# yamiel-abreu/distributed-pytorch-training

Hardware: AMD Instinct MI355X
Metric: images/sec (whole node) ResNet-50 bf16 training (higher is better)
Workload: dtype bf16

## Files before the change

csrc/bindings.cpp:

```cpp
#include <ATen/ATen.h>
#include <c10/hip/HIPGuard.h>
#include <c10/hip/HIPStream.h>
#include <torch/extension.h>

#include "kernels/kernels.h"
#include "host_comm.h"
#include "pg_comm.h"
#include "rccl_comm.h"
#include "watchdog.h"
#include "reducer.h"

namespace py = pybind11;
using at::Tensor;

namespace {

hipStream_t cur_stream(const Tensor& t) {
  return c10::hip::getCurrentHIPStream(t.device().index()).stream();
}

dpt::WireType wire_of(const Tensor& t) {
  switch (t.scalar_type()) {
    case at::kFloat: return dpt::WireType::kF32;
    case at::kBFloat16: return dpt::WireType::kBF16;
// ... 1216 lines not shown
  m.def("bias_grad16", &bias_grad16, py::arg("grad"), py::arg("out_kind"));
  m.def("sum_partials", &sum_partials, py::arg("part"), py::arg("out_kind"));
  m.def("colsum_rows", &colsum_rows, py::arg("part"), py::arg("out_kind"));
  m.def("maxpool_fwd", &maxpool_fwd, py::arg("x"), py::arg("k"), py::arg("stride"), py::arg("pad"),
        py::arg("bn_coef") = py::none());
  m.def("gap_bwd", &gap_bwd, py::arg("g"), py::arg("H"), py::arg("W"), py::arg("dtype"));
  m.def("gap_bwd_bnr", &gap_bwd_bnr, py::arg("g"), py::arg("y"), py::arg("x"), py::arg("mean"));
  m.def("maxpool_bwd", &maxpool_bwd, py::arg("grad_output"), py::arg("idx"), py::arg("H"), py::arg("W"),
        py::arg("k"), py::arg("stride"), py::arg("pad"), py::arg("grad_output2") = py::none(),
        py::arg("bn_x") = py::none(), py::arg("bn_mean") = py::none(), py::arg("bn_coef") = py::none());
  m.def("conv_fwd", &conv_fwd, py::arg("x"), py::arg("w"), py::arg("stride"), py::arg("pad"), py::arg("want_stats"),
        py::arg("out_h") = 0, py::arg("out_w") = 0);
  m.def("space_to_depth2", &space_to_depth2, py::arg("x"), py::arg("out_f16") = false);
  m.def("conv_wgrad", &conv_wgrad, py::arg("grad_output"), py::arg("x"), py::arg("weight_shape"), py::arg("stride"),
        py::arg("pad"), py::arg("fp32_out"), py::arg("target_blocks") = 0);
  m.def("conv_f32_fwd", &conv_f32_fwd, py::arg("x"), py::arg("w"), py::arg("stride"), py::arg("pad"),
        py::arg("split") = false);
  m.def("conv_f32_dgrad", &conv_f32_dgrad, py::arg("grad_output"), py::arg("w"), py::arg("stride"), py::arg("pad"),
        py::arg("H"), py::arg("W"), py::arg("split") = false);
  m.def("conv_f32_wgrad", &conv_f32_wgrad, py::arg("grad_output"), py::arg("x"), py::arg("weight_shape"),
        py::arg("stride"), py::arg("pad"), py::arg("split") = false);
  m.def("im2col", &im2col, py::arg("x"), py::arg("R"), py::arg("S"), py::arg("stride"), py::arg("pad"), py::arg("Kp"));
  m.def("attn_fwd", &attn_fwd, py::arg("qkv"), py::arg("heads"), py::arg("scale"));
  m.def("attn_set_bwd_split", &dpt::attn_set_bwd_split, py::arg("on"));
  m.def("attn_bwd", &attn_bwd, py::arg("qkv"), py::arg("out"), py::arg("grad_output"), py::arg("lse"),
        py::arg("heads"), py::arg("scale"));
  m.def("attn_stream_fwd", &attn_stream_fwd, py::arg("qkv"), py::arg("heads"), py::arg("scale"));
  m.def("attn_stream_bwd", &attn_stream_bwd, py::arg("qkv"), py::arg("out"), py::arg("grad_output"), py::arg("lse"),
        py::arg("heads"), py::arg("scale"));
  m.def("attn_stream_tiles", &attn_stream_tiles,
        "(queries per workgroup, keys per chunk, query rows per backward chunk) of the streaming attention kernels");
  m.def("conv_set_variant", &dpt::conv_set_variant, py::arg("variant"));
  m.def("bn_set_skip_finalize", &dpt::bn_set_skip_finalize, py::arg("on"),
        "measurement only: skip every BatchNorm finalize launch (wrong values; timing upper bound)");
  m.def("conv_set_splitk_policy", &dpt::conv_set_splitk_policy, py::arg("tiles"), py::arg("eager_tiles"),
        py::arg("eager_min_k"), py::arg("target"), "split-K thresholds (A/B knob; <= 0 keeps a value)");
  m.def("conv_set_big", &dpt::conv_set_big, py::arg("on"));
  m.def("conv_set_halo", &dpt::conv_set_halo, py::arg("on"));
  m.def("conv_set_breg", &dpt::conv_set_breg, py::arg("mode"));
  m.def("conv_set_wgrad_stages", &dpt::conv_set_wgrad_stages, py::arg("mode"));
  m.def("conv_get_breg", &dpt::conv_get_breg);
  m.def("conv_set_streamk", &dpt::conv_set_streamk, py::arg("mode"), py::arg("eff") = 0.0);
  m.def("conv_get_streamk", &dpt::conv_get_streamk);
  m.def("conv_sk_prepare", &dpt::conv_sk_prepare);
  m.def("conv_sk_errors", &dpt::conv_sk_errors);
  m.def("conv_sk_blocks", &dpt::conv_sk_blocks, py::arg("tiles"), py::arg("nk"), py::arg("bn"), py::arg("mode"));
  m.def("conv_set_wgrad_target", &dpt::conv_set_wgrad_target, py::arg("blocks"));
  m.def("conv_set_wgrad_halo", &dpt::conv_set_wgrad_halo, py::arg("mode"));
  m.def("conv_fwd_splits", [](int64_t M, int Cout, int64_t K, bool graph) {
          return dpt::conv_fwd_splits_for(M, Cout, K, graph);
        }, py::arg("M"), py::arg("Cout"), py::arg("K"), py::arg("graph") = false);
  m.def("conv_set_splitk", &dpt::conv_set_splitk, py::arg("mode"));
  m.def("conv_get_splitk", &dpt::conv_get_splitk);
  m.def("conv_set_fwd_shape_policy", &dpt::conv_set_fwd_shape_policy, py::arg("bits"));
  m.def("conv_dgrad", &conv_dgrad, py::arg("grad_output"), py::arg("w"), py::arg("pad"));
  m.def("conv_dgrad_bnstats", &conv_dgrad_bnstats, py::arg("grad_output"), py::arg("w"), py::arg("pad"),
        py::arg("bn_x"), py::arg("bn_mean"), py::arg("bn_coef"), py::arg("bn_y") = py::none(),
        py::arg("bn_res") = py::none(), py::arg("w_flipped") = py::none(), py::arg("bn_x2") = py::none(),
        py::arg("bn_mean2") = py::none(), py::arg("wgrad_reduce") = nullptr, py::arg("bn_mask") = py::none(),
        py::arg("bn_res_s2") = false);
  m.def("conv_wt_flip_multi", &conv_wt_flip_multi, py::arg("ws"));
  m.def("conv_dgrad_preflipped", &conv_dgrad_preflipped, py::arg("grad_output"), py::arg("w_flipped"), py::arg("pad"),
        py::arg("wgrad_reduce") = nullptr);
  m.def("bn_bwd_partials", &bn_bwd_partials, py::arg("grad_output"), py::arg("x"), py::arg("weight"), py::arg("mean"),
        py::arg("invstd"), py::arg("coef"), py::arg("p1"), py::arg("p2"), py::arg("want_dparams"),
        py::arg("from_dz") = false);
  m.def("conv_dgrad_s2", &conv_dgrad_s2, py::arg("grad_output"), py::arg("w"), py::arg("pad"), py::arg("H"),
        py::arg("W"), py::arg("bn_x") = py::none(), py::arg("bn_mean") = py::none(), py::arg("bn_coef") = py::none(),
        py::arg("wgrad_reduce") = nullptr, py::arg("compact") = false);
  m.def("conv_dgrad_flip", &conv_dgrad_flip, py::arg("grad_output"), py::arg("w"), py::arg("pad"),
        py::arg("wgrad_reduce") = nullptr);
  py::class_<PendingReduce, PendingReducePtr>(m, "PendingWgradReduce")
      .def_property_readonly("done", &PendingReduce::done)
      .def_property_readonly("splits", [](const PendingReduce& p) { return p.r.splits; });
  m.def("conv_wgrad_deferred", &conv_wgrad_deferred, py::arg("grad_output"), py::arg("x"), py::arg("weight_shape"),
        py::arg("stride"), py::arg("pad"));
  m.def("conv_reduce_flush", &conv_reduce_flush, py::arg("pending"));
  m.def("rccl_version", []() { return std::string(dpt::rccl_version_string()); });

  py::class_<dpt::Collective, std::shared_ptr<dpt::Collective>>(m, "Collective")
      .def("all_reduce", [](dpt::Collective& c, Tensor t, bool on_current_stream) {
             TORCH_CHECK(t.is_cuda() && t.is_contiguous(), "all_reduce needs a contiguous GPU tensor");
             c10::hip::HIPGuard guard(t.device().index());
             hipStream_t s = cur_stream(t);
             c.all_reduce(t.data_ptr(), (size_t)t.numel(), wire_of(t), on_current_stream ? s : c.stream());
           }, py::arg("tensor"), py::arg("on_current_stream") = true)
      .def("broadcast", [](dpt::Collective& c, Tensor t, int root) {
             TORCH_CHECK(t.is_cuda() && t.is_contiguous(), "broadcast needs a contiguous GPU tensor");
             c10::hip::HIPGuard guard(t.device().index());
             c.broadcast(t.data_ptr(), (size_t)t.numel(), wire_of(t), root, cur_stream(t));
           }, py::arg("tensor"), py::arg("root") = 0)
      .def("abort", &dpt::Collective::abort)
      .def("destroy", &dpt::Collective::destroy)
      .def("check", &dpt::Collective::check)
      .def_property_readonly("kind", &dpt::Collective::kind)
      .def_property_readonly("ops", &dpt::Collective::ops)
      .def_property_readonly("sequence_hash", &dpt::Collective::sequence_hash)
      .def_property_readonly("rank", &dpt::Collective::rank)
      .def_property_readonly("world_size", &dpt::Collective::world_size)
      .def_property_readonly("device", &dpt::Collective::device)
      .def("track", [](dpt::Collective& c) {
             c10::hip::HIPGuard guard(c.device());
             c.track(c10::hip::getCurrentHIPStream(c.device()).stream());
           }, "hand the watchdog a completion marker for the work enqueued on the current stream")
      .def("_test_spin", [](dpt::Collective& c, double ms, bool on_current_stream) {
             TORCH_CHECK(ms >= 0 && ms <= 20000, "spin: 0..20000 ms");
// ... 87 lines not shown
```

csrc/kernels/conv_kernels.hip:

```cpp
#include <algorithm>
#include <cmath>
#include <cstdlib>
#include <mutex>
#include <stdexcept>
#include <type_traits>

#include "carry.h"
#include "gelu.h"
#include "common.h"
#include "kernels.h"
#include "mfma.h"

namespace dpt {


#ifndef DPT_WGRAD_WAVES
#define DPT_WGRAD_WAVES 4
#endif
#ifndef DPT_CONV_HALF_EPI
#define DPT_CONV_HALF_EPI 0
#endif

namespace conv {

// ... 29 lines not shown
}
template <bool F16>
__device__ __forceinline__ uint32_t cpack(f32x2_t v) {
  if constexpr (F16) return __builtin_bit_cast(uint32_t, __builtin_convertvector(v, f16x2_t));
  else return __builtin_bit_cast(uint32_t, __builtin_convertvector(v, bf16x2_t));
}
template <bool F16>
__device__ __forceinline__ float cunpack(uint32_t u, int h) {
  if constexpr (F16) return (float)__builtin_bit_cast(_Float16, (uint16_t)(h ? (u >> 16) : (u & 0xffffu)));
  else return __uint_as_float(h ? (u & 0xffff0000u) : (u << 16));
}

struct ConvSk {
  float* part = nullptr;
  unsigned* flags = nullptr;
  unsigned* err = nullptr;
  int G = 0;
  uint32_t part_bytes = 0;
};

struct ConvFwdArgs {
  const uint16_t* x = nullptr;
  const uint16_t* w = nullptr;
  uint16_t* y = nullptr;
  float* psum = nullptr;
  float* psq = nullptr;
  int N = 0, H = 0, W = 0, C = 0, Ho = 0, Wo = 0, Cout = 0, R = 0, S = 0, stride = 0, pad = 0;
  int64_t M = 0;
  int m_tiles = 0, n_tiles = 0;
  int mt256 = 0;
  const uint16_t* bnx = nullptr;
  const float* bn_mean = nullptr;
  const float* bn_coef = nullptr;
  float* bp1 = nullptr;
  float* bp2 = nullptr;
  const uint16_t* bny = nullptr;
  const uint16_t* bnres = nullptr;
  const uint8_t* bnmask = nullptr;
  int rHo = 0, rWo = 0;
  const uint16_t* bias16 = nullptr;
  const uint16_t* bnx2 = nullptr;
  const float* bn_mean2 = nullptr;
  float* bp3 = nullptr;
  int Rw = 0, Sw = 0, tr0 = 0, trs = 0, ts0 = 0, tss = 0;
  int oH = 0, oW = 0, oph = 0, opw = 0;
  int bp_ld = 0, bp_off = 0;
  int f16 = 0;
  float* part = nullptr;
  int splits = 1, kps = 0;
  ReduceCarry red;
  ConvSk sk;
};


template <int N>
__device__ __forceinline__ void vmcnt_wait() {
  asm volatile("s_waitcnt vmcnt(%0)" ::"n"(N) : "memory");
}

template <int RB>
__device__ __forceinline__ bf16x8_t wg_frag(const unsigned char* img, int krow0, int col0, int lane) {
  return tr_frag<RB, false>(img, krow0, col0, lane);
}

__device__ __attribute__((aligned(64))) uint4 g_conv_zero16[4];

template <int BMT, int BN, int STAGES, bool LDSEPI, bool BKN, bool STATS = true, bool BNB = false,
          bool BNR = false, bool REMAP = false, bool ZSIB = false, bool BNR2 = false, bool F16 = false,
          int NT = conv::kThreads, bool SPLIT = false, bool HALO = false, int HB = 1, bool SK = false,
          bool DGELU = false, bool BREG = false, bool RS2 = false>
__global__ __launch_bounds__(NT, (SK || BREG) ? 4 : 2) void conv_fwd_kernel(ConvFwdArgs p) {
  static_assert(!RS2 || (BNR && !BNR2 && !REMAP && LDSEPI && !HALO && !BREG), "RS2 config");
  using namespace conv;
  constexpr int BM = BMT;
  constexpr int NW = NT / 64;
  constexpr int WCOL = BREG ? 32 : 64;
  constexpr int WN = BN / WCOL;
  constexpr int WM = NW / WN;
  constexpr int MI = BM / (WM * 32);
  constexpr int NI = WCOL / 32;
  static_assert(WM * WN == NW && MI >= 1 && MI * WM * 32 == BM, "conv_fwd_kernel: bad wave tiling");
  constexpr int A_PER_T = BM * 8 / NT;
  constexpr int B_PER_T = BN * 8 / NT;
  static_assert(!HALO || (BMT == 128 && STAGES == 1 && !BKN && !SPLIT && NT == conv::kThreads), "HALO config");
  static_assert(!SK || (STAGES == 1 && !HALO && !SPLIT && LDSEPI && !BNR2 && NT == conv::kThreads), "SK config");
  static_assert(!DGELU || (BNB && !BNR && !STATS && !REMAP && LDSEPI && !SK), "DGELU config");
  static_assert(!BREG || (BMT == 128 && STAGES == 1 && LDSEPI && !BKN && !SPLIT && !SK && HB == 1 &&
                          NT == conv::kThreads && (BN == 128 || BN == 64)), "BREG config");
  constexpr int HROWS = 136;
  static_assert(HB == 1 || (HALO && HB == 3), "HB");
  constexpr int A_BYTES = (HALO ? HROWS : BM) * kRowBytes, B_BYTES = BN * kRowBytes;
  constexpr int STAGE = A_BYTES + (BREG ? 0 : HB * B_BYTES);
  constexpr int NSTAGE = BREG ? 2 : STAGES;
  constexpr int C_STRIDE = BN * 2 + 16;
  constexpr int RED = 2 * WM * BN * 4;
  constexpr int ZROW = NSTAGE * STAGE;
  constexpr int LDS_MAIN = NSTAGE * STAGE + (HALO ? kRowBytes : 0);
  constexpr bool HALF = DPT_CONV_HALF_EPI && LDSEPI && BM == 128 && NT == conv::kThreads && MI * 32 <= 64 && !BNB &&
                        !SPLIT;
  constexpr int EROWS = HALF ? 64 : BM;
  constexpr int LDS_EPI = (LDSEPI ? EROWS * C_STRIDE : 0) + RED;
  constexpr int LDS = LDS_MAIN > LDS_EPI ? LDS_MAIN : LDS_EPI;
  __shared__ __attribute__((aligned(16))) unsigned char lds[LDS];
  if constexpr (NT == conv::kThreads) {
    if (p.red.blocks) {
      const int nconv = (int)gridDim.x - p.red.blocks;
      if ((int)blockIdx.x >= nconv) {
        carry_reduce(p.red, (int)blockIdx.x - nconv, lds);
        return;
      }
    }
  }

  const int tid = threadIdx.x, lane = tid & 63, wid = tid >> 6;
  const int wm = wid / WN, wn = wid % WN;
  const int tiles = (BM == 256 ? p.mt256 : p.m_tiles) * p.n_tiles;
  const int nk_all = (int)((int64_t)p.R * p.S * p.C / BK);

  auto tile_body = [&](const int mt, const int nt, const int sp, const int ks0, const int ks1, const int sk_role,
                       const int sk_slot, const int sk_c0, const int sk_c1) {
  const int tid = SK ? conv::opaque_v((int)threadIdx.x) : (int)threadIdx.x, lane = tid & 63;
  const int wid = SK ? __builtin_amdgcn_readfirstlane(tid >> 6) : tid >> 6;
  const int wm = wid / WN, wn = wid % WN;
  const int64_t m0 = (int64_t)mt * BM;
  const int n0 = nt * BN;

  int hi0[A_PER_T], wi0[A_PER_T], aoff[A_PER_T];
  const int64_t HoWo = (int64_t)p.Ho * p.Wo;
#pragma unroll
  for (int i = 0; i < A_PER_T; ++i) {
    const int arow = (wid * A_PER_T + i) * 8 + (lane >> 3);
    const int achunk = (lane & 7) ^ ((arow >> 1) & 7);
    const int64_t m = m0 + arow;
    if (m < p.M) {
      const int64_t n = m / HoWo;
      const int rem = (int)(m - n * HoWo);
      const int ho = rem / p.Wo, wo = rem - ho * p.Wo;
      hi0[i] = ho * p.stride - p.pad;
      wi0[i] = wo * p.stride - p.pad + (p.C < BK ? achunk * 8 / p.C : 0);
      aoff[i] = (int)(((n * p.H + hi0[i]) * (int64_t)p.W + wo * p.stride - p.pad) * p.C + achunk * 8);
    } else {
      hi0[i] = -(1 << 28);
      wi0[i] = 0;
      aoff[i] = 0;
    }
  }
  const int64_t Kg = (int64_t)p.R * p.S * p.C;
  int woff[B_PER_T];
  constexpr int RBK = BN * 2;
  constexpr int KN_RPI = 1024 / RBK;
#pragma unroll
  for (int i = 0; i < B_PER_T; ++i) {
    if (BKN) {
      const int krow = (wid * B_PER_T + i) * KN_RPI + lane / (RBK / 16);
      const int kchunk = wg_slot<RBK>(krow, lane % (RBK / 16));
      woff[i] = krow * p.Rw * p.Sw * p.Cout + n0 + kchunk * 8;
    } else {
      const int brow = (wid * B_PER_T + i) * 8 + (lane >> 3);
      const int bchunk = (lane & 7) ^ ((brow >> 1) & 7);
      woff[i] = (int)((n0 + brow) * Kg) + bchunk * 8;
    }
  }
  constexpr uint32_t kOOB = 0xFFFFFF00u;
  const __amdgpu_buffer_rsrc_t rx = __builtin_amdgcn_make_buffer_rsrc(
// ... 652 lines not shown
      if (tid < BN) {
        float a = 0.f, b = 0.f, c3 = 0.f;
#pragma unroll
        for (int w = 0; w < NW; ++w) {
          a += bred[(w * NS3) * BN + tid];
          b += bred[(w * NS3 + 1) * BN + tid];
          if (two) c3 += bred[(w * NS3 + 2) * BN + tid];
        }
        constexpr int SUBB = BM / 128;
        const int64_t pc = DGELU ? (int64_t)mt * p.Cout + n0 + tid
                                 : (int64_t)(n0 + tid) * p.bp_ld + p.bp_off + (int64_t)mt * SUBB;
        p.bp1[pc] = a;
        if (!DGELU) p.bp2[pc] = b;
        if (two) p.bp3[pc] = c3;
        if (SUBB == 2 && ((int64_t)mt * 2 + 1) * 128 < p.M) {
          p.bp1[pc + 1] = 0.f;
          if (!DGELU) p.bp2[pc + 1] = 0.f;
          if (two) p.bp3[pc + 1] = 0.f;
        }
      }
    }
  }
  };

  if constexpr (SK) {
    const uint32_t g = (uint32_t)p.sk.G >> 3, nk = (uint32_t)nk_all;
    const uint32_t x = blockIdx.x & 7, i = blockIdx.x >> 3;
    const uint32_t t_lo = (uint32_t)tiles * x / 8, t_hi = (uint32_t)tiles * (x + 1) / 8;
    const uint32_t I = (t_hi - t_lo) * nk;
    const uint32_t s0 = I * i / g, s1 = I * (i + 1) / g;
    const uint32_t f1 = min(s1, (s0 / nk + 1) * nk);
    const uint32_t nseg = s1 > s0 ? 1u + (s1 > f1 ? (s1 - 1) / nk - f1 / nk + 1 : 0u) : 0u;
    for (uint32_t q = 0; q < nseg; ++q) {
      const uint32_t b0 = q + 1 == nseg ? s0 : f1 + q * nk;
      const uint32_t tl = b0 / nk;
      const uint32_t b1 = min(s1, (tl + 1) * nk);
      const int k0 = (int)(b0 - tl * nk), k1 = (int)(b1 - tl * nk);
      int role = 0, c0 = 0, c1 = -1;
      if (k0 > 0 && k1 == nk_all) {
        role = 2;
        const uint32_t it0 = tl * nk;
        uint32_t c = it0 * g / I;
        while (c + 1 < i && I * (c + 1) / g <= it0) ++c;
        while (c > 0 && I * c / g > it0) --c;
        c0 = (int)(x + 8 * c);
        c1 = (int)blockIdx.x - 8;
      } else if (k1 < nk_all) {
        role = 1;
      }
      if (q > 0) __syncthreads();
      const int t = (int)(t_lo + tl);
      tile_body(t / p.n_tiles, t % p.n_tiles, 0, k0, k1, role, (int)blockIdx.x, c0, c1);
    }
  } else {
    const int nsplit = SPLIT ? p.splits : 1;
    const int bid0 = conv::xcd_remap(blockIdx.x, tiles * nsplit);
    const int sp = SPLIT ? bid0 % nsplit : 0;
    const int bid = SPLIT ? bid0 / nsplit : bid0;
    const int ks0 = SPLIT ? sp * p.kps : 0;
    const int ks1 = SPLIT ? min(nk_all, ks0 + p.kps) : nk_all;
    tile_body(bid / p.n_tiles, bid % p.n_tiles, sp, ks0, ks1, 0, 0, 0, -1);
  }
}

constexpr int kSplitRows = 16;
template <bool STATS, bool BNB, bool BNR, bool BNR2, bool REMAP, bool ZSIB, bool F16, bool RS2 = false>
__global__ __launch_bounds__(256) void conv_split_epilogue_kernel(ConvFwdArgs p) {
  static_assert(!RS2 || (BNR && !BNR2 && !REMAP), "RS2 config");
  const int rb = blockIdx.x, cgb = blockIdx.y, cols = gridDim.x;
  const int tid = threadIdx.x, lane = tid & 63, wid = tid >> 6;
  const int oc = tid & 7, orow = (tid >> 3) & 15, half = tid >> 7;
  const int c0 = cgb * 64 + oc * 8;
  const int64_t MC = p.M * p.Cout;
  const int64_t m = (int64_t)rb * kSplitRows + orow;
  const bool live = m < p.M;
  const int64_t poff = (live ? m : 0) * p.Cout + c0;
  int64_t grow = live ? m : 0;
  int oy = 0, ox = 0;
  if (REMAP) {
    const int64_t hw = (int64_t)p.Ho * p.Wo, img = grow / hw, rem = grow - img * hw;
    const int a = (int)(rem / p.Wo), b = (int)(rem - (int64_t)a * p.Wo);
    oy = 2 * a + p.oph;
    ox = 2 * b + p.opw;
    grow = (img * p.oH + oy) * p.oW + ox;
  }
  const int64_t off = grow * p.Cout + c0;
  float v[8];
#pragma unroll
  for (int k = 0; k < 8; ++k) v[k] = 0.f;
  if (live) {
    for (int sp = half; sp < p.splits; sp += 2) {
      const float4* q = reinterpret_cast<const float4*>(p.part + sp * MC + poff);
      const float4 a = q[0], b = q[1];
      v[0] += a.x; v[1] += a.y; v[2] += a.z; v[3] += a.w; v[4] += b.x; v[5] += b.y; v[6] += b.z; v[7] += b.w;
    }
  }
  __shared__ float join[128][9];
  __shared__ float red[2][3][64];
  if (half == 1) {
#pragma unroll
    for (int k = 0; k < 8; ++k) join[tid & 127][k] = v[k];
  }
  __syncthreads();
  constexpr bool two = BNR && BNR2;
  float q0[8], q1[8], q2[8];
#pragma unroll
// ... 892 lines not shown
}

int conv_m_tiles(int64_t M) { return (int)((M + conv::BM - 1) / conv::BM); }
int conv_split_cols(int64_t M) { return (int)((M + 15) / 16); }

static int g_conv_variant = 0;
void conv_set_variant(int v) { g_conv_variant = v; }
static int fwd_variant() { return g_conv_variant >= 20 ? 0 : g_conv_variant; }

static int g_conv_big = 0;
void conv_set_big(int on) { g_conv_big = on; }

static int g_conv_halo = 1;
void conv_set_halo(int on) { g_conv_halo = on; }

static int g_conv_breg = 0;
void conv_set_breg(int mode) { g_conv_breg = mode; }
int conv_get_breg() { return g_conv_breg; }

static int g_conv_sk = 0;
static double kSkEff = 0.9;
void conv_set_streamk(int mode, double eff) {
  g_conv_sk = mode;
  if (eff > 0) kSkEff = eff;
}
int conv_get_streamk() { return g_conv_sk; }

static int g_splitk = 1;
void conv_set_splitk(int mode) { g_splitk = mode; }
int conv_get_splitk() { return g_splitk; }
static int kSplitTiles = 160, kSplitEager = 32, kSplitTarget = 512, kSplitEagerMinK = 24;
void conv_set_splitk_policy(int tiles, int eager_tiles, int eager_min_k, int target) {
  if (tiles > 0) kSplitTiles = tiles;
  if (eager_tiles > 0) kSplitEager = eager_tiles;
  if (eager_min_k > 0) kSplitEagerMinK = eager_min_k;
  if (target > 0) kSplitTarget = target;
}

static int g_fwd_shape_policy = 0;
void conv_set_fwd_shape_policy(int bits) { g_fwd_shape_policy = bits; }

static int g_wgrad_halo = 5;
void conv_set_wgrad_halo(int on) { g_wgrad_halo = on; }

static int g_wgrad_target = 0;
void conv_set_wgrad_target(int blocks) { g_wgrad_target = blocks; }

static int g_wgrad_stages = 0;
void conv_set_wgrad_stages(int mode) { g_wgrad_stages = mode; }

enum : unsigned {
  kLdsEpi = 1u << 0, kBkn = 1u << 1, kStats = 1u << 2, kBnb = 1u << 3, kBnr = 1u << 4, kRemap = 1u << 5,
  kZsib = 1u << 6, kBnr2 = 1u << 7, kF16 = 1u << 8, kSplit = 1u << 9, kHalo = 1u << 10, kSk = 1u << 11,
  kDgelu = 1u << 12, kBreg = 1u << 13, kDir = 1u << 14, kRs2 = 1u << 15,
};
static constexpr bool has(unsigned flags, unsigned f) { return (flags & f) != 0; }
static constexpr unsigned opt(bool on, unsigned f) { return on ? f : 0u; }
template <unsigned F>
using Opts = std::integral_constant<unsigned, F>;

template <class Fn>
static void with_bool(bool b, Fn&& fn) {
  if (b) fn(std::true_type{});
  else fn(std::false_type{});
}

template <int BMT, int BN, int STAGES, unsigned F, int NT = conv::kThreads, int HB = 1>
static void launch_fwd_kernel(dim3 grid, hipStream_t s, const ConvFwdArgs& a) {
  hipLaunchKernelGGL((conv_fwd_kernel<BMT, BN, STAGES, has(F, kLdsEpi), has(F, kBkn), has(F, kStats), has(F, kBnb),
                                      has(F, kBnr), has(F, kRemap), has(F, kZsib), has(F, kBnr2), has(F, kF16), NT,
                                      has(F, kSplit), has(F, kHalo), HB, has(F, kSk), has(F, kDgelu), has(F, kBreg),
                                      has(F, kRs2)>),
                     grid, dim3(NT), 0, s, a);
}

template <unsigned F>
static void launch_split_epilogue_kernel(dim3 grid, hipStream_t s, const ConvFwdArgs& a) {
  hipLaunchKernelGGL((conv_split_epilogue_kernel<has(F, kStats), has(F, kBnb), has(F, kBnr), has(F, kBnr2),
                                                 has(F, kRemap), has(F, kZsib), has(F, kF16), has(F, kRs2)>),
                     grid, dim3(256), 0, s, a);
}

template <int BMW, int BNW, int STAGES, unsigned F, int NT = conv::kThreads>
static void launch_wgrad_kernel(dim3 grid, hipStream_t s, const ConvWgradArgs& a) {
  hipLaunchKernelGGL((conv_wgrad_kernel<BMW, BNW, STAGES, has(F, kF16), NT, has(F, kDir)>), grid, dim3(NT), 0, s, a);
}

template <int BNW, int STAGES, unsigned F>
static void launch_wgrad_halo_kernel(dim3 grid, hipStream_t s, const ConvWgradArgs& a) {
  hipLaunchKernelGGL((conv_wgrad_halo_kernel<BNW, STAGES, has(F, kF16)>), grid, dim3(conv::kThreads), 0, s, a);
}

static int conv_big_auto(int64_t M, int N, int64_t K, int taps) {
  if (!g_conv_big) return 0;
  if (g_conv_big >= 2) {
    const int64_t kmin = g_conv_big == 2 ? 1024 : 512;
    return (taps == 1 && K >= kmin && N % 256 == 0) ? 13 : 0;
  }
  if (N == 256 && K >= 1024 && M >= 32768) return 9;
  if (N == 512 && K >= 2048 && M <= 16384) return 10;
  return 0;
}

static void conv_check_offsets(const ConvFwdArgs& a, bool bkn) {
  const int64_t xb = (int64_t)a.N * a.H * a.W * a.C * 2;
  const int64_t wb = (int64_t)(bkn ? a.Rw * a.Sw : a.R * a.S) * a.C * a.Cout * 2;
  if (xb >= 0xFFFFFF00ll || wb >= 0x7FFFFFFFll)
    throw std::runtime_error("conv: operand tensors beyond 2^31 elements are not supported");
}

static thread_local WgradReduce* g_attached_reduce = nullptr;

static int reduce_phases(int splits) { return splits >= 16 ? 16 : splits >= 4 ? 4 : 1; }

void launch_wgrad_reduce(const WgradReduce& r, hipStream_t st) {
  const float4* part = reinterpret_cast<const float4*>(r.part);
  const int ph = reduce_phases(r.splits), out_per_block = kBlock / ph;
  const dim3 grid((unsigned)((r.n4 + out_per_block - 1) / out_per_block)), block(kBlock);
  if (ph == 16) hipLaunchKernelGGL(conv_wgrad_reduce_kernel<16>, grid, block, 0, st, part, r.n4, r.splits, r.out, r.kind);
  else if (ph == 4) hipLaunchKernelGGL(conv_wgrad_reduce_kernel<4>, grid, block, 0, st, part, r.n4, r.splits, r.out, r.kind);
  else hipLaunchKernelGGL(conv_wgrad_reduce_kernel<1>, grid, block, 0, st, part, r.n4, r.splits, r.out, r.kind);
}

AttachWgradReduce::AttachWgradReduce(WgradReduce* r, hipStream_t s) : r_(r), s_(s) {
  if (g_attached_reduce != nullptr) throw std::runtime_error("AttachWgradReduce: a reduce is already attached");
// ... 365 lines not shown
void launch_conv_dgrad(const uint16_t* dy, const uint16_t* w, uint16_t* dx, int N, int Ho, int Wo, int Cout, int C,
                       int R, int S, int pad, hipStream_t s, bool f16) {
  conv_fwd_impl(dy, w, dx, N, Ho, Wo, Cout, C, R, S, 1, R - 1 - pad, nullptr, nullptr, true, s, 0, 0, f16);
}

struct S2Class {
  int ph, pw, Rc, Sc, pad, Ha, Wa, tr0, ts0;
  bool zsib;
};
static int s2_classes(int H, int W, int R, int S, int pad, S2Class* out) {
  int J[2], r0[2], Js[2], s0[2], D[2];
  for (int ph = 0; ph < 2; ++ph) {
    r0[ph] = ((ph + pad) % 2 + 2) % 2;
    J[ph] = r0[ph] < R ? (R - 1 - r0[ph]) / 2 + 1 : 0;
    D[ph] = (ph + pad - r0[ph]) / 2;
    s0[ph] = r0[ph];
    Js[ph] = s0[ph] < S ? (S - 1 - s0[ph]) / 2 + 1 : 0;
  }
  const bool zsib = J[1] == 0 && Js[1] == 0 && J[0] > 0 && Js[0] > 0;
  int n = 0;
  for (int ph = 0; ph < 2; ++ph)
    for (int pw = 0; pw < 2; ++pw) {
      const int Ha = (H - ph + 1) / 2, Wa = (W - pw + 1) / 2;
      if (Ha <= 0 || Wa <= 0 || J[ph] == 0 || Js[pw] == 0) continue;
      const int pad_c = J[ph] - 1 - D[ph];
      if (Js[pw] - 1 - D[pw] != pad_c) throw std::runtime_error("conv_dgrad_s2: unequal class paddings");
      out[n++] = S2Class{ph, pw, J[ph], Js[pw], pad_c, Ha, Wa, r0[ph] + 2 * (J[ph] - 1), s0[pw] + 2 * (Js[pw] - 1),
                         zsib && ph == 0 && pw == 0};
    }
  return n;
}

ConvS2Plan conv_dgrad_s2_plan(int N, int H, int W, int C, int Cout, int R, int S, int pad, hipStream_t s) {
  S2Class cl[4];
  const int n = s2_classes(H, W, R, S, pad, cl);
  ConvS2Plan pl{0, 0};
  for (int i = 0; i < n; ++i) {
    const int64_t M = (int64_t)N * cl[i].Ha * cl[i].Wa;
    const int splits = conv_fwd_splits(M, C, (int64_t)cl[i].Rc * cl[i].Sc * Cout, nullptr, s);
    pl.chunks += splits > 1 ? conv_split_cols(M) : conv_m_tiles(M);
    if (splits > 1) pl.ws_floats = std::max(pl.ws_floats, (int64_t)splits * M * C);
  }
  return pl;
}

int conv_dgrad_s2_chunks(int N, int H, int W, int R, int S, int pad) {
  S2Class cl[4];
  const int n = s2_classes(H, W, R, S, pad, cl);
  int chunks = 0;
  for (int i = 0; i < n; ++i) chunks += conv_m_tiles((int64_t)N * cl[i].Ha * cl[i].Wa);
  return chunks;
}

void launch_conv_dgrad_s2(const uint16_t* dy, const uint16_t* w, uint16_t* dx, int N, int Ho, int Wo, int Cout,
                          int C, int R, int S, int pad, int H, int W, hipStream_t s, const uint16_t* bnx,
                          const float* bn_mean, const float* bn_coef, float* bp1, float* bp2, bool f16, float* ws,
                          bool compact) {
  const bool bnb = bnx != nullptr;
  const int bp_ld = bnb ? (ws ? conv_dgrad_s2_plan(N, H, W, C, Cout, R, S, pad, s).chunks
                              : conv_dgrad_s2_chunks(N, H, W, R, S, pad))
                        : 0;
  int bp_off = 0;
  S2Class cl[4];
  const int ncl = s2_classes(H, W, R, S, pad, cl);
  if (compact && (bnb || ncl != 1 || !cl[0].zsib))
    throw std::runtime_error("conv_dgrad_s2: the compact gradient needs a 1x1 kernel and no BN statistics");
  for (int ci = 0; ci < ncl; ++ci) {
    const S2Class& k = cl[ci];
    ConvFwdArgs a = conv_args(dy, w, dx, f16, N, Ho, Wo, Cout, C, k.Rc, k.Sc, 1, k.pad, k.Ha, k.Wa);
    a.Rw = R; a.Sw = S;
    a.tr0 = k.tr0; a.trs = -2;
    a.ts0 = k.ts0; a.tss = -2;
    a.oH = H; a.oW = W; a.oph = k.ph; a.opw = k.pw;
    a.bnx = bnx; a.bn_mean = bn_mean; a.bn_coef = bn_coef;
    a.bp1 = bp1; a.bp2 = bp2; a.bp_ld = bp_ld; a.bp_off = bp_off;
    if (bnb && k.zsib) throw std::runtime_error("conv_dgrad_s2: BN statistics with zero-filled classes unsupported");
    const auto run = [&](auto epi) {
      constexpr unsigned F = kBkn | decltype(epi)::value;
      if (maybe_split<F>(a, ws, s)) {
        bp_off += conv_split_cols(a.M);
        return;
      }
      bp_off += a.m_tiles;
      fwd_launch_default<F>(a, s);
    };
    if (compact) run(Opts<0u>{});
    else if (bnb) run(Opts<kRemap | kBnb>{});
    else if (k.zsib) run(Opts<kRemap | kZsib>{});
    else run(Opts<kRemap>{});
  }
}

static int wgrad_halo_mode(int C) {
  if (g_wgrad_halo == 5) return C == 64 ? 3 : 0;
  if (g_wgrad_halo == 6) return C == 64 ? 4 : 0;
  return g_wgrad_halo;
}

static FastDiv make_fastdiv(uint32_t d) {
  FastDiv f;
  f.d = d;
  if (d <= 1) { f.mul = 0; f.shr = 0; return f; }
  uint32_t l = 0;
  while ((1ull << l) < d) ++l;
  f.mul = (uint32_t)(((1ull << (31 + l)) + d - 1) / d);
  f.shr = l - 1;
  return f;
}

static int wgrad_target(int R, int S, int stride, int steps) {
  if (g_wgrad_target > 0) return g_wgrad_target;
  if (R * S == 1 && stride == 1) return 512;
  return steps >= 3136 ? 768 : 640;
}

ConvWgradPlan conv_wgrad_plan(int N, int H, int W, int C, int Cout, int R, int S, int stride, int pad, int Ho,
                              int Wo, int target_blocks) {
  ConvWgradPlan pl;
  pl.Ho = Ho > 0 ? Ho : (H + 2 * pad - R) / stride + 1;
  pl.Wo = Wo > 0 ? Wo : (W + 2 * pad - S) / stride + 1;
  const int64_t M = (int64_t)N * pl.Ho * pl.Wo;
  const int hmode = wgrad_halo_mode(C);
  if (hmode && R == 3 && S == 3 && stride == 1 && pad == 1 && pl.Ho == H && pl.Wo == W &&
      C % (hmode >= 3 ? 64 : 128) == 0 && Cout % 64 == 0 && (int64_t)N * H * (W + 2) + 128 < (1ll << 31)) {
    pl.halo = hmode;
    pl.bmw = 64;
    pl.bnw = pl.halo >= 3 ? 64 : 128;
    const int tiles = (Cout / 64) * 3 * (C / pl.bnw);
// ... 107 lines not shown
```

csrc/kernels/kernels.h:

```cpp
#pragma once

#include <hip/hip_runtime.h>
#include <stdint.h>

namespace dpt {

struct AugNorm {
  float mean[4];
  float inv_std[4];
};

void launch_grad_check(const float* g, int64_t n, const float* scale, float host_factor,
                       float* found_inf, hipStream_t s);
void launch_sgd(float* p, float* g, float* buf, int64_t n, float lr, float momentum,
                float dampening, float wd, bool nesterov, const float* scale, float host_factor,
                const float* found_inf, const float* step, bool zero_grad, uint16_t* shadow,
                int shadow_kind, hipStream_t s);
void launch_adam(float* p, float* g, float* m, float* v, int64_t n, double lr, double beta1,
                 double beta2, double eps, double wd, bool adamw, const float* scale, float host_factor,
                 const float* found_inf, const float* step, bool zero_grad, uint16_t* shadow,
                 int shadow_kind, hipStream_t s);
void launch_optim_tail(float* scale, int* growth_tracker, float* found_inf, float* step,
                       float growth_factor, float backoff_factor, int growth_interval,
                       hipStream_t s);
// ... 63 lines not shown
  float* dst[kGatherMax];
  int64_t numel[kGatherMax];
  int8_t kind[kGatherMax];
  int count;
};
void launch_gather(const GatherBatch& batch, bool accumulate, hipStream_t s);

bool ln_supported(int64_t D);
int ln_bwd_blocks(int64_t T);
int gelu_bwd_chunks(int64_t T, int64_t F);
void vit_set_gelu_blocks_per_cu(int n);
void launch_ln_fwd(int kind, const float* x, const uint16_t* a, const void* bias, int bias_kind, const float* gamma,
                   const float* beta, float* s_out, uint16_t* h_out, float* mean, float* rstd, int64_t T, int64_t D,
                   float eps, hipStream_t s);
void launch_ln_bwd(int kind, const float* gs, const uint16_t* gh, const float* sv, const float* mean,
                   const float* rstd, const float* gamma, float* gx, uint16_t* ga, float* part, float* dgamma,
                   float* dbeta, void* dbias, int dbias_kind, int64_t T, int64_t D, hipStream_t s);
void launch_gelu_fwd(int kind, const uint16_t* u, const void* bias, int bias_kind, uint16_t* h, int64_t T, int64_t F,
                     hipStream_t s);
void launch_gelu_bwd(int kind, const uint16_t* gh, const uint16_t* u, const void* bias, int bias_kind, uint16_t* gu,
                     float* part, void* dbias, int dbias_kind, int64_t T, int64_t F, hipStream_t s);
void launch_bias_grad16(int kind, const uint16_t* gy, float* part, void* dbias, int dbias_kind, int64_t T, int64_t F,
                        hipStream_t s);
void launch_sum_partials(const float* part, int64_t n, int S, void* out, int out_kind, hipStream_t s);
void launch_colsum_rows(const float* part, int64_t n, int64_t D, void* out, int out_kind, hipStream_t s);
void launch_rows_copy16(const uint16_t* src, uint16_t* dst, const int n[4], const int64_t ss[4], const int64_t ds[4],
                        int L, hipStream_t s);

bool conv_supported(int C, int Cout);
bool conv_supported_narrow(int C, int Cout, int S);
int conv_m_tiles(int64_t M);
void conv_set_variant(int v);
void conv_set_big(int on);
void conv_set_wgrad_stages(int mode);
void conv_set_breg(int mode);
int conv_get_breg();
void conv_set_halo(int on);
void launch_linear_dgrad_dgelu(const uint16_t* dy, const uint16_t* wt, const uint16_t* u, const float* bias,
                               const uint16_t* bias16, uint16_t* gu, float* bp1, int64_t T, int n_out, int n_in,
                               bool f16, hipStream_t s);
int linear_dgrad_dgelu_tiles(int64_t T);
void conv_set_streamk(int mode, double eff);
int conv_get_streamk();
void conv_sk_prepare();
unsigned conv_sk_errors();
int conv_sk_blocks(int64_t tiles, int nk, int bn, int mode);
void conv_set_wgrad_target(int blocks);
int conv_fwd_splits(int64_t M, int Cout, int64_t K, int* kps = nullptr, hipStream_t s = nullptr);
int conv_fwd_splits_for(int64_t M, int Cout, int64_t K, bool graph, int* kps = nullptr);
int conv_split_cols(int64_t M);
void conv_set_splitk_policy(int tiles, int eager_tiles, int eager_min_k, int target);
void conv_set_splitk(int mode);
int conv_get_splitk();
void conv_set_fwd_shape_policy(int bits);
void launch_conv_fwd(const uint16_t* x, const uint16_t* w, uint16_t* y, int N, int H, int W, int C, int Cout,
                     int R, int S, int stride, int pad, float* psum, float* psq, hipStream_t s, int Ho = 0,
                     int Wo = 0, bool f16 = false, float* ws = nullptr);
struct ConvWgradPlan {
  int Ho, Wo, bmw, bnw, splits, steps_per_split;
  int64_t part_floats;
  int halo = 0;
};
void conv_set_wgrad_halo(int mode);
ConvWgradPlan conv_wgrad_plan(int N, int H, int W, int C, int Cout, int R, int S, int stride, int pad, int Ho = 0,
                              int Wo = 0, int target_blocks = 0);
struct WgradReduce {
  const float* part;
  void* out;
  int64_t n4;
  int splits, kind;
  bool consumed;
};
void launch_wgrad_reduce(const WgradReduce& r, hipStream_t s);
void launch_conv_wgrad(const uint16_t* dy, const uint16_t* x, float* part, void* dw, int dw_kind, int N, int H,
                       int W, int C, int Cout, int R, int S, int stride, int pad, const ConvWgradPlan& plan,
                       hipStream_t s, bool f16 = false, WgradReduce* defer = nullptr);
void launch_bn_bwd_apply_pre(int dtype, const void* dy, const void* x, int64_t M, int64_t C, const float* mean,
                             const float* coef, const float* kbuf, void* dx, hipStream_t s, bool from_dz);
struct ReduceCarry;
int take_attached_reduce(ReduceCarry& rc);
class AttachWgradReduce {
 public:
  AttachWgradReduce(WgradReduce* r, hipStream_t s);
  ~AttachWgradReduce();
  AttachWgradReduce(const AttachWgradReduce&) = delete;
  AttachWgradReduce& operator=(const AttachWgradReduce&) = delete;

 private:
  WgradReduce* r_;
  hipStream_t s_;
};
void launch_conv_dgrad_bnstats(const uint16_t* dy, const uint16_t* wt, uint16_t* dx, int N, int Ho, int Wo, int Cout,
                               int C, int R, int S, int pad, const uint16_t* bnx, const float* bn_mean,
                               const float* bn_coef, float* bp1, float* bp2, hipStream_t s,
                               const uint16_t* bny = nullptr, const uint16_t* bnres = nullptr,
                               const uint16_t* bnx2 = nullptr, const float* bn_mean2 = nullptr,
                               float* bp3 = nullptr, bool f16 = false, float* ws = nullptr,
                               const uint8_t* bnmask = nullptr, bool res_s2 = false);
constexpr int kWtFlipMax = 64;
struct WtFlipBatch {
  const uint16_t* w[kWtFlipMax];
  uint16_t* wt[kWtFlipMax];
  int Cout[kWtFlipMax], R[kWtFlipMax], S[kWtFlipMax], C[kWtFlipMax];
  int blk0[kWtFlipMax];
  int count;
};
// ... 43 lines not shown
```

distributed_pytorch_training_amd/ops/conv.py:

```python
from __future__ import annotations

import os

import torch

from . import native, native_available

_CL = torch.channels_last
_DT16 = (torch.bfloat16, torch.float16)
ENABLED = os.environ.get("DPT_NATIVE_CONV", "1") != "0"
BN_BWD_FUSE = os.environ.get("DPT_BN_BWD_FUSE", "1") != "0"
_BNB_PARTIALS = {}
_GEN = [0]
S2_DGRAD = os.environ.get("DPT_S2_DGRAD", "1") != "0"
S2_COMPACT_DRES = os.environ.get("DPT_S2_COMPACT_DRES", "1") != "0"
WGRAD_REDUCE_FUSE = os.environ.get("DPT_WGRAD_REDUCE_FUSE", "1") != "0"
STEM_ENABLED = os.environ.get("DPT_NATIVE_STEM", "0") == "1"


MIN_PIXELS = int(os.environ.get("DPT_CONV_MIN_PIXELS", "0"))


def supported(x: torch.Tensor, w: torch.Tensor, stride, padding, dilation, groups, min_pixels=None) -> bool:
    if not (ENABLED and x.is_cuda and native_available() and x.dtype in _DT16
            and w.dtype == x.dtype and x.dim() == 4 and groups == 1):
        return False
    if tuple(dilation) != (1, 1) or stride[0] != stride[1] or padding[0] != padding[1]:
        return False
    cout, cin, r, s = w.shape
    ho = (x.shape[2] + 2 * padding[0] - r) // stride[0] + 1
    wo = (x.shape[3] + 2 * padding[1] - s) // stride[1] + 1
    return (cin % 64 == 0 and cout % 64 == 0 and r == s and x.shape[1] == cin
            and x.shape[0] * ho * wo >= (MIN_PIXELS if min_pixels is None else min_pixels)
            and x.is_contiguous(memory_format=_CL))


def _cl(t: torch.Tensor) -> torch.Tensor:
    return t if t.is_contiguous(memory_format=_CL) else t.contiguous(memory_format=_CL)


_CALLS = None


def profile_calls(on: bool) -> None:
    global _CALLS
    _CALLS = [] if on else None


def take_profile():
    out = list(_CALLS or [])
    if _CALLS is not None:
        _CALLS.clear()
    return out


def _mark():
    if _CALLS is None:
        return None
    e = torch.cuda.Event(enable_timing=True)
    e.record()
    return e


def _note(kind, x, w, stride, pad, variant, e0, out_hw=(0, 0)):
    if _CALLS is None or e0 is None:
        return
    co, ci, r, _ = w.shape
    key = (ci, x.shape[2], x.shape[3], co, r, int(stride), int(pad), tuple(int(v) for v in out_hw))
    _CALLS.append((kind, key, variant, e0, _mark()))


def _backward(ctx, dy):
    x, w = ctx.saved_tensors
    dy = _cl(dy.to(x.dtype))
    s, p = ctx.stride, ctx.pad
    dx = dw = red = None
    e0 = _mark()
    if ctx.needs_input_grad[1]:
        if ctx.needs_input_grad[0] and WGRAD_REDUCE_FUSE:
            dw, red = native().conv_wgrad_deferred(dy, x, list(w.shape), s, p)
        else:
            dw = native().conv_wgrad(dy, x, list(w.shape), s, p, False)
        _note("wgrad", x, w, s, p, "deferred-reduce" if red is not None else "reduce", e0)
        e0 = _mark()
    variant = None
    if ctx.needs_input_grad[0]:
        src = ctx.bn_src if (s == 1 and BN_BWD_FUSE) else None
        dres = None
        wt = _flipped(w) if s == 1 else None
        slot = ctx.bn_src[2] if (ctx.bn_src is not None and isinstance(ctx.bn_src[2], dict)) else None
        compact = False
        if slot is not None:
            slot.pop("fold_s2", None)
            compact = bool(slot.pop("dres_s2", False))
            if compact and not (src is not None and len(src) == 3 and _is_compact_of(slot.get("dres"), x)):
                raise RuntimeError("fused block-tail backward: a downsample conv handed over a compact "
                                   "identity-path gradient that this conv's backward-data cannot fold")
        if src is not None and not isinstance(src[2], dict):
            bn_x, bn_mean, bn_coef = src
            dx, p1, p2, _ = native().conv_dgrad_bnstats(dy, w, p, bn_x, bn_mean, bn_coef, w_flipped=wt,
                                                        wgrad_reduce=red)
            _put_bnb(dx, p1, p2, None, None)
            variant = "bnrelu-stats"
        elif (src is not None and _dres_ok(dres := src[2].pop("dres", None), x)
              and (compact or dres.shape == x.shape)):
            bn_x, bn_mean = src[0], src[1]
            x2, mean2 = (src[3], src[4]) if len(src) > 3 else (None, None)
            dx, p1, p2, p3 = native().conv_dgrad_bnstats(dy, w, p, bn_x, bn_mean, None, x, dres, wt, x2, mean2,
                                                         wgrad_reduce=red, bn_mask=src[2].get("mask"),
                                                         bn_res_s2=compact)
            _put_bnb(dx, p1, p2, COMPACT_RES if compact else dres.data_ptr(), p3 if x2 is not None else None)
            variant = "tail-stats-s2res" if compact else "tail+ds-stats" if x2 is not None else "tail-stats"
        elif s == 1:
            dx = (native().conv_dgrad_flip(dy, w, p, wgrad_reduce=red)[0] if wt is None
                  else native().conv_dgrad_preflipped(dy, wt, p, wgrad_reduce=red))
            variant = "plain"
        elif s == 2 and S2_DGRAD and x.dim() == 4:
            src = ctx.bn_src if BN_BWD_FUSE else None
            rs = ctx.res_slot
            if (ctx.compact_dres and S2_COMPACT_DRES and BN_BWD_FUSE and rs is not None and rs.get("fold_s2")
                    and "dres" not in rs):
                rs["dres"] = native().conv_dgrad_s2(dy, w, p, x.shape[2], x.shape[3], wgrad_reduce=red,
                                                    compact=True)[0]
                rs["dres_s2"] = True
                variant = "s2-compact"
            elif src is not None and not isinstance(src[2], dict) and w.shape[2] > 1:
                dx, p1, p2 = native().conv_dgrad_s2(dy, w, p, x.shape[2], x.shape[3], src[0], src[1], src[2],
                                                    wgrad_reduce=red)
                _put_bnb(dx, p1, p2, None, None)
                variant = "s2-bnrelu-stats"
            else:
                dx = native().conv_dgrad_s2(dy, w, p, x.shape[2], x.shape[3], wgrad_reduce=red)[0]
                variant = "s2"
        else:
            dx = torch.ops.aten.convolution_backward(dy, x, w, None, (s, s), (p, p), (1, 1), False, (0, 0), 1,
                                                     (True, False, False))[0]
    if red is not None and not red.done:
        native().conv_reduce_flush(red)
    if variant is not None:
        _note("dgrad", x, w, s, p, variant + ("+reduce" if red is not None else ""), e0)
    if variant == "s2-compact":
        return None, dw
    if dx is not None and ctx.res_slot is not None:
        ctx.res_slot["dres"] = dx
    return dx, dw


_FLIP = {"on": False, "pending": {}, "done": {}}


def reset_side_channels() -> None:
    _GEN[0] += 1
    _BNB_PARTIALS.clear()


def _put_bnb(dx, p1, p2, dres_ptr, p3) -> None:
    _BNB_PARTIALS[dx.data_ptr()] = (_GEN[0], dx._version, p1, p2, tuple(dx.shape), dres_ptr, p3)


def begin_step() -> None:
    reset_side_channels()
    _FLIP["on"] = True
    _FLIP["pending"].clear()
    _FLIP["done"].clear()


def end_caching() -> None:
    _FLIP["on"] = False
    _FLIP["pending"].clear()
    _FLIP["done"].clear()


# ... 144 lines not shown
```

Before: 12930.

## Group stride-2 dgrad phase classes into a single grouped kernel launch

Stride-2 dgrad is decomposed into up to four phase classes, each previously launched as its own conv kernel. This adds a GROUP variant of the forward conv kernel that takes per-class parameters and maps each block to a class, m-tile and n-tile, so all classes run in one launch with classes sorted by kernel size. The goal is fewer launches and better GPU fill for small per-class grids. It is only used when no split-K or stream-K applies, and blocks beyond a class's m-tile count exit early, which can waste some grid slots.

```diff
diff --git a/csrc/bindings.cpp b/csrc/bindings.cpp
--- a/csrc/bindings.cpp
+++ b/csrc/bindings.cpp
@@ -1292,6 +1292,8 @@
         }, py::arg("M"), py::arg("Cout"), py::arg("K"), py::arg("graph") = false);
   m.def("conv_set_splitk", &dpt::conv_set_splitk, py::arg("mode"));
   m.def("conv_get_splitk", &dpt::conv_get_splitk);
+  m.def("conv_set_s2_group", &dpt::conv_set_s2_group, py::arg("on"));
+  m.def("conv_s2_group_launches", &dpt::conv_s2_group_launches);
   m.def("conv_set_fwd_shape_policy", &dpt::conv_set_fwd_shape_policy, py::arg("bits"));
   m.def("conv_dgrad", &conv_dgrad, py::arg("grad_output"), py::arg("w"), py::arg("pad"));
   m.def("conv_dgrad_bnstats", &conv_dgrad_bnstats, py::arg("grad_output"), py::arg("w"), py::arg("pad"),
diff --git a/csrc/kernels/conv_kernels.hip b/csrc/kernels/conv_kernels.hip
--- a/csrc/kernels/conv_kernels.hip
+++ b/csrc/kernels/conv_kernels.hip
@@ -105,6 +105,15 @@
   ConvSk sk;
 };
 
+struct ConvGrpClass {
+  int R = 0, S = 0, pad = 0, Ho = 0, Wo = 0, m_tiles = 0, tr0 = 0, ts0 = 0, oph = 0, opw = 0, bp_off = 0;
+  int64_t M = 0;
+};
+struct ConvGrpArgs : ConvFwdArgs {
+  ConvGrpClass cls[4];
+  int ncls = 0, mt_max = 0;
+};
+
 
 template <int N>
 __device__ __forceinline__ void vmcnt_wait() {
@@ -121,9 +130,12 @@
 template <int BMT, int BN, int STAGES, bool LDSEPI, bool BKN, bool STATS = true, bool BNB = false,
           bool BNR = false, bool REMAP = false, bool ZSIB = false, bool BNR2 = false, bool F16 = false,
           int NT = conv::kThreads, bool SPLIT = false, bool HALO = false, int HB = 1, bool SK = false,
-          bool DGELU = false, bool BREG = false, bool RS2 = false>
-__global__ __launch_bounds__(NT, (SK || BREG) ? 4 : 2) void conv_fwd_kernel(ConvFwdArgs p) {
+          bool DGELU = false, bool BREG = false, bool RS2 = false, bool GROUP = false>
+__global__ __launch_bounds__(NT, (SK || BREG) ? 4 : 2) void conv_fwd_kernel(
+    std::conditional_t<GROUP, ConvGrpArgs, ConvFwdArgs> p) {
   static_assert(!RS2 || (BNR && !BNR2 && !REMAP && LDSEPI && !HALO && !BREG), "RS2 config");
+  static_assert(!GROUP || (BKN && REMAP && LDSEPI && !ZSIB && !BNR && !SPLIT && !HALO && !SK && !BREG && BMT == 128 &&
+                         STAGES == 1 && NT == conv::kThreads), "GROUP config");
   using namespace conv;
   constexpr int BM = BMT;
   constexpr int NW = NT / 64;
@@ -163,6 +175,21 @@
         return;
       }
     }
+  }
+
+  int grp_mt = 0, grp_nt = 0;
+  if constexpr (GROUP) {
+    const int per = p.ncls * p.n_tiles;
+    const int t = conv::xcd_remap(blockIdx.x, p.mt_max * per);
+    grp_mt = t / per;
+    const int rem = t - grp_mt * per, ci = rem / p.n_tiles;
+    grp_nt = rem - ci * p.n_tiles;
+#define DPT_GRP_PICK(f) p.f = ci == 0 ? p.cls[0].f : ci == 1 ? p.cls[1].f : ci == 2 ? p.cls[2].f : p.cls[3].f
+    DPT_GRP_PICK(R); DPT_GRP_PICK(S); DPT_GRP_PICK(pad); DPT_GRP_PICK(Ho); DPT_GRP_PICK(Wo); DPT_GRP_PICK(m_tiles);
+    DPT_GRP_PICK(tr0); DPT_GRP_PICK(ts0); DPT_GRP_PICK(oph); DPT_GRP_PICK(opw); DPT_GRP_PICK(bp_off);
+    DPT_GRP_PICK(M);
+#undef DPT_GRP_PICK
+    if (grp_mt >= p.m_tiles) return;
   }
 
   const int tid = threadIdx.x, lane = tid & 63, wid = tid >> 6;
@@ -921,6 +948,8 @@
       const int t = (int)(t_lo + tl);
       tile_body(t / p.n_tiles, t % p.n_tiles, 0, k0, k1, role, (int)blockIdx.x, c0, c1);
     }
+  } else if constexpr (GROUP) {
+    tile_body(grp_mt, grp_nt, 0, 0, nk_all, 0, 0, 0, -1);
   } else {
     const int nsplit = SPLIT ? p.splits : 1;
     const int bid0 = conv::xcd_remap(blockIdx.x, tiles * nsplit);
@@ -1919,7 +1948,7 @@
 enum : unsigned {
   kLdsEpi = 1u << 0, kBkn = 1u << 1, kStats = 1u << 2, kBnb = 1u << 3, kBnr = 1u << 4, kRemap = 1u << 5,
   kZsib = 1u << 6, kBnr2 = 1u << 7, kF16 = 1u << 8, kSplit = 1u << 9, kHalo = 1u << 10, kSk = 1u << 11,
-  kDgelu = 1u << 12, kBreg = 1u << 13, kDir = 1u << 14, kRs2 = 1u << 15,
+  kDgelu = 1u << 12, kBreg = 1u << 13, kDir = 1u << 14, kRs2 = 1u << 15, kGrp = 1u << 16,
 };
 static constexpr bool has(unsigned flags, unsigned f) { return (flags & f) != 0; }
 static constexpr unsigned opt(bool on, unsigned f) { return on ? f : 0u; }
@@ -1933,11 +1962,12 @@
 }
 
 template <int BMT, int BN, int STAGES, unsigned F, int NT = conv::kThreads, int HB = 1>
-static void launch_fwd_kernel(dim3 grid, hipStream_t s, const ConvFwdArgs& a) {
+static void launch_fwd_kernel(dim3 grid, hipStream_t s,
+                              const std::conditional_t<has(F, kGrp), ConvGrpArgs, ConvFwdArgs>& a) {
   hipLaunchKernelGGL((conv_fwd_kernel<BMT, BN, STAGES, has(F, kLdsEpi), has(F, kBkn), has(F, kStats), has(F, kBnb),
                                       has(F, kBnr), has(F, kRemap), has(F, kZsib), has(F, kBnr2), has(F, kF16), NT,
                                       has(F, kSplit), has(F, kHalo), HB, has(F, kSk), has(F, kDgelu), has(F, kBreg),
-                                      has(F, kRs2)>),
+                                      has(F, kRs2), has(F, kGrp)>),
                      grid, dim3(NT), 0, s, a);
 }
 
@@ -2409,6 +2439,23 @@
   return chunks;
 }
 
+static int g_s2_group = 1;
+static int64_t g_s2_group_launches = 0;
+void conv_set_s2_group(int on) { g_s2_group = on; }
+int64_t conv_s2_group_launches() { return g_s2_group_launches; }
+
+template <unsigned E>
+static void s2_group_launch(ConvGrpArgs& g, hipStream_t s) {
+  g.n_tiles = g.Cout % 128 == 0 ? g.Cout / 128 : g.Cout / 64;
+  const dim3 grid((unsigned)(g.mt_max * g.ncls * g.n_tiles + take_attached_reduce(g.red)));
+  with_bool(g.Cout % 128 == 0, [&](auto wide) {
+    with_bool(g.f16, [&](auto f16) {
+      launch_fwd_kernel<128, wide.value ? 128 : 64, 1, kLdsEpi | kBkn | kGrp | E | opt(f16.value, kF16)>(grid, s, g);
+    });
+  });
+  ++g_s2_group_launches;
+}
+
 void launch_conv_dgrad_s2(const uint16_t* dy, const uint16_t* w, uint16_t* dx, int N, int Ho, int Wo, int Cout,
                           int C, int R, int S, int pad, int H, int W, hipStream_t s, const uint16_t* bnx,
                           const float* bn_mean, const float* bn_coef, float* bp1, float* bp2, bool f16, float* ws,
@@ -2422,15 +2469,44 @@
   const int ncl = s2_classes(H, W, R, S, pad, cl);
   if (compact && (bnb || ncl != 1 || !cl[0].zsib))
     throw std::runtime_error("conv_dgrad_s2: the compact gradient needs a 1x1 kernel and no BN statistics");
-  for (int ci = 0; ci < ncl; ++ci) {
-    const S2Class& k = cl[ci];
+  const auto class_args = [&](const S2Class& k, int off) {
     ConvFwdArgs a = conv_args(dy, w, dx, f16, N, Ho, Wo, Cout, C, k.Rc, k.Sc, 1, k.pad, k.Ha, k.Wa);
     a.Rw = R; a.Sw = S;
     a.tr0 = k.tr0; a.trs = -2;
     a.ts0 = k.ts0; a.tss = -2;
     a.oH = H; a.oW = W; a.oph = k.ph; a.opw = k.pw;
     a.bnx = bnx; a.bn_mean = bn_mean; a.bn_coef = bn_coef;
-    a.bp1 = bp1; a.bp2 = bp2; a.bp_ld = bp_ld; a.bp_off = bp_off;
+    a.bp1 = bp1; a.bp2 = bp2; a.bp_ld = bp_ld; a.bp_off = off;
+    return a;
+  };
+  bool group = g_s2_group && !compact && ncl >= 2 && !g_conv_sk;
+  for (int ci = 0; group && ws != nullptr && ci < ncl; ++ci)
+    group = conv_fwd_splits((int64_t)N * cl[ci].Ha * cl[ci].Wa, C, (int64_t)cl[ci].Rc * cl[ci].Sc * Cout, nullptr,
+                            s) <= 1;
+  if (group) {
+    int order[4] = {0, 1, 2, 3};
+    std::stable_sort(order, order + ncl, [&](int i, int j) { return cl[i].Rc * cl[i].Sc > cl[j].Rc * cl[j].Sc; });
+    int off[4];
+    for (int ci = 0; ci < ncl; ++ci) {
+      off[ci] = bp_off;
+      bp_off += conv_m_tiles((int64_t)N * cl[ci].Ha * cl[ci].Wa);
+    }
+    ConvGrpArgs g;
+    g.ncls = ncl;
+    for (int q = 0; q < ncl; ++q) {
+      const ConvFwdArgs a = class_args(cl[order[q]], off[order[q]]);
+      conv_check_offsets(a, true);
+      if (q == 0) static_cast<ConvFwdArgs&>(g) = a;
+      g.cls[q] = ConvGrpClass{a.R, a.S, a.pad, a.Ho, a.Wo, a.m_tiles, a.tr0, a.ts0, a.oph, a.opw, a.bp_off, a.M};
+      g.mt_max = std::max(g.mt_max, a.m_tiles);
+    }
+    if (bnb) s2_group_launch<kRemap | kBnb>(g, s);
+    else s2_group_launch<kRemap>(g, s);
+    return;
+  }
+  for (int ci = 0; ci < ncl; ++ci) {
+    const S2Class& k = cl[ci];
+    ConvFwdArgs a = class_args(k, bp_off);
     if (bnb && k.zsib) throw std::runtime_error("conv_dgrad_s2: BN statistics with zero-filled classes unsupported");
     const auto run = [&](auto epi) {
       constexpr unsigned F = kBkn | decltype(epi)::value;
diff --git a/csrc/kernels/kernels.h b/csrc/kernels/kernels.h
--- a/csrc/kernels/kernels.h
+++ b/csrc/kernels/kernels.h
@@ -139,6 +139,8 @@
 void conv_set_splitk_policy(int tiles, int eager_tiles, int eager_min_k, int target);
 void conv_set_splitk(int mode);
 int conv_get_splitk();
+void conv_set_s2_group(int on);
+int64_t conv_s2_group_launches();
 void conv_set_fwd_shape_policy(int bits);
 void launch_conv_fwd(const uint16_t* x, const uint16_t* w, uint16_t* y, int N, int H, int W, int C, int Cout,
                      int R, int S, int stride, int pad, float* psum, float* psq, hipStream_t s, int Ho = 0,
diff --git a/distributed_pytorch_training_amd/ops/conv.py b/distributed_pytorch_training_amd/ops/conv.py
--- a/distributed_pytorch_training_amd/ops/conv.py
+++ b/distributed_pytorch_training_amd/ops/conv.py
@@ -14,6 +14,7 @@
 _GEN = [0]
 S2_DGRAD = os.environ.get("DPT_S2_DGRAD", "1") != "0"
 S2_COMPACT_DRES = os.environ.get("DPT_S2_COMPACT_DRES", "1") != "0"
+S2_GROUP = os.environ.get("DPT_S2_GROUP", "1") != "0"
 WGRAD_REDUCE_FUSE = os.environ.get("DPT_WGRAD_REDUCE_FUSE", "1") != "0"
 STEM_ENABLED = os.environ.get("DPT_NATIVE_STEM", "0") == "1"
 
@@ -118,6 +119,7 @@
         elif s == 2 and S2_DGRAD and x.dim() == 4:
             src = ctx.bn_src if BN_BWD_FUSE else None
             rs = ctx.res_slot
+            native().conv_set_s2_group(int(bool(S2_GROUP)))
             if (ctx.compact_dres and S2_COMPACT_DRES and BN_BWD_FUSE and rs is not None and rs.get("fold_s2")
                     and "dres" not in rs):
                 rs["dres"] = native().conv_dgrad_s2(dy, w, p, x.shape[2], x.shape[3], wgrad_reduce=red,
```

Result: no change. 12870 (-0.5%).
